# xh92117/Retinex-image-Enhancement

Hardware: AMD Instinct MI355X
Metric: images/sec at 512x512 bs=32 per GPU (UP-Retinex forward) (higher is better)
Workload: dtype f32; 1 GPU; configs[1]: bs=32/GPU 512x512 plain forward, fp32; global_batch=32, image_size=512, variant=plain, parallelism=batch-shard x1 (no data-path collective)

## Files before the change

### retinex-image-enhancement_amd/csrc/conv_ring.hip

```cpp
#include <algorithm>
#include <cstdlib>
#include <cstring>

#include "upr_common.h"

namespace upr {

typedef float f32x4_r __attribute__((ext_vector_type(4)));
typedef _Float16 f16x8_r __attribute__((ext_vector_type(8)));
typedef _Float16 f16x4_r __attribute__((ext_vector_type(4)));
typedef __attribute__((address_space(3))) void* lds_void_ptr_r;

__device__ __attribute__((aligned(256))) uint4 g_ring_zero[16];
__device__ __attribute__((aligned(256))) uint2 g_ring_sink[512 * 16];
__device__ __attribute__((aligned(256))) float g_ring_sink32[512 * 64];
__device__ __attribute__((aligned(256))) unsigned g_ring_ninf32[64] = {
#define NINF4 0xFF800000u, 0xFF800000u, 0xFF800000u, 0xFF800000u
    NINF4, NINF4, NINF4, NINF4, NINF4, NINF4, NINF4, NINF4, NINF4, NINF4, NINF4, NINF4, NINF4, NINF4, NINF4, NINF4
#undef NINF4
};
__device__ __attribute__((aligned(256))) unsigned g_ring_ninf[64] = {
#define NINF4 0xFC00FC00u, 0xFC00FC00u, 0xFC00FC00u, 0xFC00FC00u
    NINF4, NINF4, NINF4, NINF4, NINF4, NINF4, NINF4, NINF4, NINF4, NINF4, NINF4, NINF4, NINF4, NINF4, NINF4, NINF4
#undef NINF4
};

enum RingMode : int { kRingConv = 0, kRingHead = 1, kRingFam = 2, kRingS2 = 3 };
enum RingFlags : int {
  kRingRes = 1, kRingRelu = 2, kRingSc = 4, kRingOcc3 = 8, kRingWide = 16, kRingOut2 = 32, kRingOut32 = 64,
  kRingDil2 = 128, kRingResPre = 256, kRingPool = 512, kRingXPool = 1024, kRingR32 = 2048,
  kRingAblDma = 4096, kRingAblMma = 8192, kRingAblSt = 16384,
  kRingMma16 = 32768
};

template <int NPL, int RW_, int GROWS_, bool DEINT_ = false>
struct Ring {
  static constexpr int RW = RW_;
  static constexpr int GROWS = GROWS_;
  static constexpr int RR = 4 * GROWS;
  static constexpr int PLANE = RR * RW * 16;
  static constexpr int BYTES = NPL * PLANE;
  static constexpr int GPX = GROWS * RW;
  static constexpr int NI = (GPX + 63) / 64;
  static constexpr int PPW = NPL / 4;
  static constexpr int G = NI * PPW;
  static constexpr bool DEINT = DEINT_;
  static constexpr int HALF = (RW + 1) / 2;
  static_assert(NPL % 4 == 0, "planes are split over the 4 waves");
  static_assert((RR & (RR - 1)) == 0, "ring rows: power of two");
};

template <class R>
struct RingLanes {
  int dr[R::NI], col[R::NI], off[R::NI];
  __device__ __forceinline__ void init(int lane, int W, int cs) {
#pragma unroll
    for (int i = 0; i < R::NI; ++i) {
      const int q = i * 64 + lane;
      const int p = q % R::RW;
      dr[i] = q < R::GPX ? q / R::RW : -1;
      col[i] = R::DEINT ? (p < R::HALF ? 2 * p : 2 * (p - R::HALF) + 1) : p;
      off[i] = (dr[i] * W + col[i]) * cs;
    }
  }
  __device__ __forceinline__ void issue(const half_t* src, int cs, int b, int H, int W, int iy0, int ix0, bool live,
                                        const half_t* fill, unsigned char* ring, int grp, int wave) const {
    const half_t* base = src + ((long long)(b * H + iy0) * W + ix0) * cs;
#pragma unroll
    for (int i = 0; i < R::NI; ++i) {
      if (dr[i] >= 0) {
        const bool ok = live && (unsigned)(iy0 + dr[i]) < (unsigned)H && (unsigned)(ix0 + col[i]) < (unsigned)W;
        const half_t* p = ok ? base + off[i] : fill;
#pragma unroll
        for (int k = 0; k < R::PPW; ++k) {
          const int c = wave + 4 * k;
          __builtin_amdgcn_global_load_lds(p + c * 8, (lds_void_ptr_r)(ring + c * R::PLANE + grp * R::GPX * 16 + i * 1024),
                                           16, 0, 0);
        }
      }
    }
  }
};
// ... 640 lines not shown
        for (int nt = 0; nt < NT; ++nt)
#pragma unroll
          for (int i = 0; i < 4; ++i) {
            float v = pool[nt][i];
            v += __shfl_xor(v, 1);
            v += __shfl_xor(v, 2);
            v += __shfl_xor(v, 4);
            v += __shfl_xor(v, 8);
            if (fr == 0) pool_add(op.pool, (size_t)b * op.N + nt * 16 + fg * 4 + i, v);
            pool[nt][i] = 0.f;
          }
        flushed = true;
      }
    }
    advance(cc);
  }
  asm volatile("s_waitcnt vmcnt(0)" ::: "memory");
}

template <int CPP>
__device__ __forceinline__ int ring32_res_swz(int l) {
  if constexpr (CPP == 8) return (l >> 1) & 7;
  else return l & 15;
}

template <int MODE, int NB, int FL>
struct Ring32Cfg {
  static constexpr bool HEAD = MODE == kRingHead;
  static constexpr bool RES = FL & kRingRes, RELU = (FL & kRingRelu) != 0;
  static constexpr bool RESPRE = (FL & kRingResPre) != 0, POOL = (FL & kRingPool) != 0;
  static constexpr int DIL = (FL & kRingDil2) ? 2 : 1, HA = DIL;
  static constexpr bool XP = (FL & kRingXPool) != 0;
  static constexpr int C = 32, NT = NB / 16, NG = 2;
  using RA = Ring<8, 32 + 2 * HA, 4>;
  using RB = Ring<8, 34, 4>;
  static constexpr int NSL = XP ? 11 : 9;
  static constexpr bool WREG = NT == 2 || (NT == 4 && !RES);
  static constexpr bool M16 = (FL & kRingMma16) != 0;
  static_assert(!M16 || WREG, "split in registers: register-resident filters only");
  static constexpr bool TAPCH = M16 && NT == 4;
  static constexpr int WBYTES = TAPCH ? 9 * NT * 1024 : WREG ? 0 : 9 * NB * 32 * 4;
  static constexpr int EW = RES ? 32 * NB * 4 : HEAD ? 512 : 0;
  static constexpr int E = RES ? NB / 8 : HEAD ? 1 : 0;
  static constexpr int LDS = WBYTES + RA::BYTES + (XP ? RB::BYTES : 0) + 4 * EW;
  static constexpr int G = RA::G + (XP ? RB::G : 0);
  static constexpr int S = HEAD ? NG : NG * NT;
  static constexpr int W0 = G, W1 = E + G + S, WK = 2 * S + E + G, WF = WK + (POOL ? 4 * NT : 0);
  static_assert(WF <= 63, "vmcnt immediate");
  static_assert(!RESPRE || RES, "kRingResPre qualifies kRingRes");
  static_assert(!(HEAD && (POOL || DIL == 2)), "head: plain 3x3");
  static_assert(!XP || (WREG && DIL == 1 && !RES && !HEAD), "x / maxpool slices: the FAM h3 part");
};

template <int MODE, int NB, int FL>
__global__ __launch_bounds__(256) void conv_ring32_kernel(RingArgs a) {
  using K = Ring32Cfg<MODE, NB, FL>;
  using RA = typename K::RA;
  constexpr bool HEAD = K::HEAD, RES = K::RES;
  constexpr int NT = K::NT, NG = K::NG, HA = K::HA, DIL = K::DIL;
  using RB = typename K::RB;
  typedef float f32x4 __attribute__((ext_vector_type(4)));
  const ConvOp& op = a.op;
  extern __shared__ __attribute__((aligned(16))) unsigned char smem[];
  unsigned char* Wl = smem;
  unsigned char* ringA = smem + K::WBYTES;
  const int tid = threadIdx.x, lane = tid & 63;
  const int wave = __builtin_amdgcn_readfirstlane(tid >> 6);
  const int fr = lane & 15, fg = lane >> 4;
  unsigned char* ringB = ringA + RA::BYTES;
  unsigned char* epi = ringA + RA::BYTES + (K::XP ? RB::BYTES : 0) + wave * K::EW;
  const int H = op.Ho, W = op.Wo;
  const ConvSeg& sa = op.seg[0];
  const int per_xcd = gridDim.x >> 3;
  const int v0 = (blockIdx.x & 7) * per_xcd + (blockIdx.x >> 3);
  const int nu = v0 < a.nunits ? (a.nunits - 1 - v0) / (int)gridDim.x + 1 : 0;
  const int KT = nu * a.steps;

  constexpr bool M16 = K::M16;
  f32x4 wr[K::WREG && !M16 ? K::NSL : 1][NT][2];
  f16x8_t wh[M16 ? K::NSL : 1][NT], wl[M16 && !K::TAPCH ? K::NSL : 1][NT];
  int wsh[NT];
  if constexpr (M16) {
#pragma unroll
    for (int nt = 0; nt < NT; ++nt) {
      const float* row = (const float*)op.W + (size_t)(nt * 16 + fr) * op.Kpad + fg * 8;
      float mx = 0.f;
#pragma unroll
      for (int t = 0; t < K::NSL; ++t) {
        const f32x4 w0 = *(const f32x4*)(row + t * 32), w1 = *(const f32x4*)(row + t * 32 + 4);
#pragma unroll
        for (int i = 0; i < 4; ++i) mx = fmaxf(mx, fmaxf(__builtin_fabsf(w0[i]), __builtin_fabsf(w1[i])));
      }
      mx = fmaxf(mx, __shfl_xor(mx, 16));
      mx = fmaxf(mx, __shfl_xor(mx, 32));
      wsh[nt] = split_row_shift(mx);
      const float wsn = __builtin_ldexpf(1.f, wsh[nt]);
#pragma unroll
      for (int t = 0; t < K::NSL; ++t) {
        const f32x4 w0 = *(const f32x4*)(row + t * 32), w1 = *(const f32x4*)(row + t * 32 + 4);
        const float v[8] = {w0[0], w0[1], w0[2], w0[3], w1[0], w1[1], w1[2], w1[3]};
        if constexpr (K::TAPCH) {
          f16x8_t lo;
          split_w_f32x8(v, wsn, wh[t][nt], lo);
          if (wave == 0) *(f16x8_t*)(Wl + (t * NT + nt) * 1024 + lane * 16) = lo;
        } else {
          split_w_f32x8(v, wsn, wh[t][nt], wl[t][nt]);
        }
      }
    }
  } else if constexpr (K::WREG) {
#pragma unroll
// ... 11 lines not shown
  }
  const half_t* srcA = (const half_t*)((const float*)sa.src + sa.coff);
  const int csA = sa.cs * 2;
  const half_t* zero = (const half_t*)g_ring_zero;
  RingLanes<RA> la;
  la.init(lane, sa.Win, csA);
  const ConvSeg& sx = op.seg[K::XP ? 1 : 0];
  const half_t* srcB = (const half_t*)((const float*)sx.src + sx.coff);
  const int csB = sx.cs * 2;
  const half_t* ninf = (const half_t*)g_ring_ninf32;
  RingLanes<RB> lb;
  if constexpr (K::XP) lb.init(lane, sx.Win, csB);

  auto unit_of = [&](int j, int& b, int& y0, int& x0) {
    const int u = v0 + j * (int)gridDim.x;
    const int sx = u % a.nstrips, r = u / a.nstrips;
    b = r / a.nseg;
    y0 = (r % a.nseg) * a.rs;
    x0 = sx * 32;
  };
  const int S = a.steps - 1;
  struct Cursor {
    int j, s, b, y0, x0;
  };
  Cursor cc{0, -1, 0, 0, 0};
  if (nu > 0) unit_of(0, cc.b, cc.y0, cc.x0);
  Cursor dc = cc;
  auto advance = [&](Cursor& c) {
    if (++c.s == S) {
      c.s = -1;
      if (++c.j < nu) unit_of(c.j, c.b, c.y0, c.x0);
    }
  };
  auto issue = [&](int k) {
    const bool live = dc.j < nu;
    la.issue(srcA, csA, dc.b, sa.Hin, sa.Win, dc.y0 + 4 * dc.s + HA, dc.x0 - HA, live, zero, ringA, (k + 1) & 3, wave);
    if constexpr (K::XP)
      lb.issue(srcB, csB, dc.b, sx.Hin, sx.Win, dc.y0 + 4 * dc.s + 1, dc.x0 - 1, live, ninf, ringB, (k + 1) & 3, wave);
    advance(dc);
  };

  __syncthreads();
  issue(0);
  issue(1);

  float bv[NT][4];
#pragma unroll
  for (int nt = 0; nt < NT; ++nt)
#pragma unroll
    for (int i = 0; i < 4; ++i) bv[nt][i] = op.bias ? op.bias[nt * 16 + fg * 4 + i] : 0.f;
  int esh[M16 ? NT : 1];
  if constexpr (M16) {
#pragma unroll
    for (int nt = 0; nt < NT; ++nt) {
      esh[nt] = 0;
#pragma unroll
      for (int i = 0; i < 4; ++i) {
        const int sh = __shfl(wsh[nt], fg * 4 + i);
        esh[nt] |= (sh & 255) << (8 * i);
        bv[nt][i] = __builtin_ldexpf(bv[nt][i], sh);
      }
    }
  }
  float bad = 0.f;
  float hw2[NT][4];
  if constexpr (HEAD) {
#pragma unroll
    for (int nt = 0; nt < NT; ++nt)
#pragma unroll
      for (int i = 0; i < 4; ++i) hw2[nt][i] = op.head_w[nt * 16 + fg * 4 + i];
  }
  const int abase = 2 * fg * RA::PLANE + fr * 16;
  const int ocs = op.out_cs, rcs = RES ? (K::RESPRE ? op.res1_cs : op.res2_cs) : 0;
  const float* resp = RES ? (const float*)(K::RESPRE ? op.res1 : op.res2) : nullptr;
  const size_t HWs = (size_t)H * W;
  float pool[K::POOL ? NT : 1][4];
#pragma unroll
  for (int nt = 0; nt < (K::POOL ? NT : 1); ++nt)
#pragma unroll
    for (int i = 0; i < 4; ++i) pool[nt][i] = 0.f;
  bool flushed = false;

  for (int kk = 0; kk < KT; ++kk) {
    if (kk == 0) asm volatile("s_waitcnt vmcnt(%0)" ::"n"(K::W0) : "memory");
    else if (kk == 1) asm volatile("s_waitcnt vmcnt(%0)" ::"n"(K::W1) : "memory");
    else if (K::POOL && flushed) asm volatile("s_waitcnt vmcnt(%0)" ::"n"(K::WF) : "memory");
    else asm volatile("s_waitcnt vmcnt(%0)" ::"n"(K::WK) : "memory");
    __builtin_amdgcn_s_barrier();
    flushed = false;
    const int s = cc.s, b = cc.b, x0 = cc.x0;
    const int yend = min(H, cc.y0 + a.rs);
    const int y = cc.y0 + 4 * s + wave;
    const bool rowok = s >= 0 && y < yend;
    const size_t prow = (size_t)(b * H + (rowok ? y : 0)) * W + x0;
    bool ovalid[NG];
#pragma unroll
    for (int g = 0; g < NG; ++g) ovalid[g] = rowok && x0 + g * 16 + fr < W;
    if constexpr (RES) {
      constexpr int CPP = NB / 4;
#pragma unroll
      for (int i = 0; i < K::E; ++i) {
        const int q = i * 64 + lane, px = q / CPP;
        const bool ok = rowok && x0 + px < W;
        const void* p = ok ? (const void*)(resp + (prow + px) * rcs + ((q % CPP) ^ ring32_res_swz<CPP>(px)) * 4)
                           : (const void*)zero;
        __builtin_amdgcn_global_load_lds(p, (lds_void_ptr_r)(epi + i * 1024), 16, 0, 0);
      }
    }
    if constexpr (HEAD) {
      const int ppc = op.x_f16 ? 8 : 4, cpr = 32 / ppc;
      if (lane < 3 * cpr) {
        const int c = lane / cpr, k = lane % cpr;
        const bool ok = rowok && x0 + k * ppc < W;
        const size_t e = (size_t)b * 2 * HWs + prow + c * HWs + k * ppc;
        const void* p = !ok ? (const void*)zero
                            : op.x_f16 ? (const void*)((const half_t*)op.x_nchw + e) : (const void*)(op.x_nchw + e);
        __builtin_amdgcn_global_load_lds(p, (lds_void_ptr_r)epi, 16, 0, 0);
      }
    }
    issue(kk + 2);

    f32x4 acc[NT][NG];
#pragma unroll
    for (int nt = 0; nt < NT; ++nt)
#pragma unroll
      for (int g = 0; g < NG; ++g) acc[nt][g] = f32x4{bv[nt][0], bv[nt][1], bv[nt][2], bv[nt][3]};
    f32x4 acc2[M16 ? NT : 1][NG];
    if constexpr (M16) {
#pragma unroll
      for (int nt = 0; nt < NT; ++nt)
#pragma unroll
        for (int g = 0; g < NG; ++g) acc2[nt][g] = f32x4{0.f, 0.f, 0.f, 0.f};
    }
    auto mm16 = [&](int t, int g, const f32x4& x0, const f32x4& x1, const f16x8_t (&wlo)[NT]) {
      const float v[8] = {x0[0], x0[1], x0[2], x0[3], x1[0], x1[1], x1[2], x1[3]};
      f16x8_t xh, xl;
      split_f32x8(v, xh, xl);
#pragma unroll
      for (int nt = 0; nt < NT; ++nt) {
        acc[nt][g] = __builtin_amdgcn_mfma_f32_16x16x32_f16(wh[t][nt], xh, acc[nt][g], 0, 0, 0);
        acc[nt][g] = __builtin_amdgcn_mfma_f32_16x16x32_f16(wlo[nt], xh, acc[nt][g], 0, 0, 0);
        acc2[nt][g] = __builtin_amdgcn_mfma_f32_16x16x32_f16(wh[t][nt], xl, acc2[nt][g], 0, 0, 0);
      }
    };
#define RING_FENCE __builtin_amdgcn_sched_barrier(0)
#define RING_LDS_DONE                                                               \
  do {                                                                              \
    RING_FENCE;                                                                     \
    __builtin_amdgcn_s_waitcnt(0xC07F);  \
    RING_FENCE;                                                                     \
  } while (0)
    constexpr bool TAPCH = K::TAPCH;
    if constexpr (TAPCH) {
      if (s >= 0) {
        static_assert(NG == 2, "chunk index: tap * 2 + group");
        f32x4 tx[2][2];
        f16x8_t wlt[2][NT];
        auto ldt = [&](int c, f32x4 (&x)[2]) {
          const int r = (c >> 1) / 3, sc = (c >> 1) % 3, g = c & 1;
          const unsigned char* xr = ringA + abase + ((4 * kk + 4 + wave - HA + (r - 1) * DIL) & 15) * (RA::RW * 16) +
                                    (g * 16 + HA + (sc - 1) * DIL) * 16;
#pragma unroll
          for (int h = 0; h < 2; ++h) x[h] = *(const f32x4*)(xr + h * RA::PLANE);
          if (g == 0) {
#pragma unroll
            for (int nt = 0; nt < NT; ++nt)
              wlt[(c >> 1) & 1][nt] = *(const f16x8_t*)(Wl + ((c >> 1) * NT + nt) * 1024 + lane * 16);
          }
        };
        auto mmt = [&](int c, const f32x4 (&x)[2]) { mm16(c >> 1, c & 1, x[0], x[1], wlt[(c >> 1) & 1]); };
        ldt(0, tx[0]);
        ldt(1, tx[1]);
        RING_LDS_DONE;
        mmt(0, tx[0]);
#pragma unroll
        for (int c = 1; c < 18; ++c) {
          RING_FENCE;
          if (c + 1 < 18) ldt(c + 1, tx[(c + 1) & 1]);
          RING_FENCE;
          mmt(c, tx[c & 1]);
          RING_LDS_DONE;
        }
      }
    }
    if (s >= 0 && !TAPCH) {
      auto rowA = [&](int r) { return ((4 * kk + 4 + wave - HA + (r - 1) * DIL) & 15) * (RA::RW * 16); };
      constexpr int NW = K::WREG ? 1 : 3;
      f32x4 bx[2][3][NG][2], bw[2][NW][NT][2];
      auto ld = [&](int r, f32x4 (&x)[3][NG][2], f32x4 (&w)[NW][NT][2]) {
        const unsigned char* xr = ringA + abase + rowA(r);
#pragma unroll
        for (int sc = 0; sc < 3; ++sc)
#pragma unroll
          for (int g = 0; g < NG; ++g)
#pragma unroll
            for (int h = 0; h < 2; ++h)
              x[sc][g][h] = *(const f32x4*)(xr + h * RA::PLANE + (g * 16 + HA + (sc - 1) * DIL) * 16);
        if constexpr (!K::WREG) {
#pragma unroll
          for (int sc = 0; sc < 3; ++sc)
#pragma unroll
            for (int nt = 0; nt < NT; ++nt)
#pragma unroll
              for (int h = 0; h < 2; ++h)
                w[sc][nt][h] = *(const f32x4*)(Wl + ((size_t)((r * 3 + sc) * NB + nt * 16 + fr) * 32 + fg * 8 + h * 4) * 4);
        }
      };
      auto mm = [&](int r, const f32x4 (&x)[3][NG][2], const f32x4 (&w)[NW][NT][2]) {
        if constexpr (M16) {
#pragma unroll
          for (int sc = 0; sc < 3; ++sc)
#pragma unroll
            for (int g = 0; g < NG; ++g) mm16(r * 3 + sc, g, x[sc][g][0], x[sc][g][1], wl[r * 3 + sc]);
          return;
        }
#pragma unroll
        for (int sc = 0; sc < 3; ++sc)
#pragma unroll
          for (int j = 0; j < 8; ++j)
#pragma unroll
            for (int g = 0; g < NG; ++g)
#pragma unroll
              for (int nt = 0; nt < NT; ++nt) {
                const float wv = K::WREG ? wr[r * 3 + sc][nt][j >> 2][j & 3] : w[K::WREG ? 0 : sc][nt][j >> 2][j & 3];
                acc[nt][g] = __builtin_amdgcn_mfma_f32_16x16x4f32(wv, x[sc][g][j >> 2][j & 3], acc[nt][g], 0, 0, 0);
              }
      };
      ld(0, bx[0], bw[0]);
      ld(1, bx[1], bw[1]);
      RING_LDS_DONE;
      mm(0, bx[0], bw[0]);
      RING_FENCE;
      ld(2, bx[0], bw[0]);
      RING_FENCE;
      mm(1, bx[1], bw[1]);
      RING_LDS_DONE;
      if constexpr (K::XP) {
        const int bbase = 2 * fg * RB::PLANE + fr * 16;
        auto rowB = [&](int dy) { return ((4 * kk + 4 + wave - 1 + dy) & 15) * (RB::RW * 16); };
        f32x4 xr3[3][NG][2];
#pragma unroll
        for (int sc = 0; sc < 3; ++sc)
#pragma unroll
          for (int g = 0; g < NG; ++g)
#pragma unroll
            for (int h = 0; h < 2; ++h)
              xr3[sc][g][h] = *(const f32x4*)(ringB + bbase + rowB(-1) + h * RB::PLANE + (g * 16 + sc) * 16);
        RING_FENCE;
        mm(2, bx[0], bw[0]);
        RING_LDS_DONE;
        f32x4 ctr[NG][2], mx[NG][2];
#pragma unroll
        for (int g = 0; g < NG; ++g)
#pragma unroll
          for (int h = 0; h < 2; ++h)
            mx[g][h] = __builtin_elementwise_max(__builtin_elementwise_max(xr3[0][g][h], xr3[1][g][h]), xr3[2][g][h]);
#pragma unroll
        for (int dr = 1; dr < 3; ++dr) {
#pragma unroll
          for (int sc = 0; sc < 3; ++sc)
#pragma unroll
            for (int g = 0; g < NG; ++g)
#pragma unroll
              for (int h = 0; h < 2; ++h)
                xr3[sc][g][h] = *(const f32x4*)(ringB + bbase + rowB(dr - 1) + h * RB::PLANE + (g * 16 + sc) * 16);
          RING_LDS_DONE;
#pragma unroll
          for (int g = 0; g < NG; ++g)
#pragma unroll
            for (int h = 0; h < 2; ++h) {
              mx[g][h] = __builtin_elementwise_max(
                  mx[g][h], __builtin_elementwise_max(__builtin_elementwise_max(xr3[0][g][h], xr3[1][g][h]), xr3[2][g][h]));
              if (dr == 1) ctr[g][h] = xr3[1][g][h];
            }
        }
        if constexpr (M16) {
#pragma unroll
          for (int g = 0; g < NG; ++g) {
            mm16(9, g, ctr[g][0], ctr[g][1], wl[K::XP ? 9 : 0]);
            mm16(10, g, mx[g][0], mx[g][1], wl[K::XP ? 10 : 0]);
          }
        } else {
#pragma unroll
        for (int j = 0; j < 8; ++j)
#pragma unroll
          for (int g = 0; g < NG; ++g)
#pragma unroll
            for (int nt = 0; nt < NT; ++nt) {
              acc[nt][g] = __builtin_amdgcn_mfma_f32_16x16x4f32(wr[9][nt][j >> 2][j & 3], ctr[g][j >> 2][j & 3],
                                                                acc[nt][g], 0, 0, 0);
              acc[nt][g] = __builtin_amdgcn_mfma_f32_16x16x4f32(wr[10][nt][j >> 2][j & 3], mx[g][j >> 2][j & 3],
                                                                acc[nt][g], 0, 0, 0);
            }
        }
      } else {
        mm(2, bx[0], bw[0]);
      }
    }
#undef RING_LDS_DONE
#undef RING_FENCE

    asm volatile("s_waitcnt vmcnt(%0)" ::"n"(K::G) : "memory");
    if constexpr (M16) {
#pragma unroll
      for (int nt = 0; nt < NT; ++nt)
#pragma unroll
        for (int g = 0; g < NG; ++g)
#pragma unroll
          for (int i = 0; i < 4; ++i) {
            const float v = __builtin_fmaf(acc2[nt][g][i], kSplitLoInv, acc[nt][g][i]);
            bad = __builtin_fmaf(ovalid[g] ? v : 0.f, 0.f, bad);
            acc[nt][g][i] = __builtin_ldexpf(v, -(int)(signed char)(esh[nt] >> (8 * i)));
          }
    }
    if constexpr (HEAD) {
#pragma unroll
      for (int g = 0; g < NG; ++g) {
        float part = 0.f;
#pragma unroll
        for (int nt = 0; nt < NT; ++nt)
#pragma unroll
          for (int i = 0; i < 4; ++i) part += fmaxf(acc[nt][g][i], 0.f) * hw2[nt][i];
        part += __shfl_xor(part, 16);
        part += __shfl_xor(part, 32);
        const int xp = g * 16 + fr;
        float x0f, x1f, x2f;
        if (op.x_f16) {
          const half_t* xl = (const half_t*)epi;
          x0f = (float)xl[xp];
          x1f = (float)xl[32 + xp];
          x2f = (float)xl[64 + xp];
        } else {
          const float* xl = (const float*)epi;
// ... 19 lines not shown
          if constexpr (K::RELU) {
#pragma unroll
            for (int i = 0; i < 4; ++i) v[i] = fmaxf(v[i], 0.f);
          }
          if constexpr (RES && !K::RESPRE)
            v += *(const f32x4*)(epi + (g * 16 + fr) * NB * 4 + (((nt * 4 + fg) ^ ring32_res_swz<NB / 4>(fr)) * 16));
          if constexpr (K::POOL) {
#pragma unroll
            for (int i = 0; i < 4; ++i)
              if (ovalid[g]) pool[nt][i] += v[i];
          }
          *(f32x4*)(dg + nt * 16) = v;
        }
      }
    }
    if constexpr (K::POOL) {
      if (s == a.steps - 2) {
#pragma unroll
        for (int nt = 0; nt < NT; ++nt)
#pragma unroll
          for (int i = 0; i < 4; ++i) {
            float v = pool[nt][i];
            v += __shfl_xor(v, 1);
            v += __shfl_xor(v, 2);
            v += __shfl_xor(v, 4);
            v += __shfl_xor(v, 8);
            if (fr == 0) pool_add(op.pool, (size_t)cc.b * op.N + nt * 16 + fg * 4 + i, v);
            pool[nt][i] = 0.f;
          }
        flushed = true;
      }
    }
    advance(cc);
  }
  asm volatile("s_waitcnt vmcnt(0)" ::: "memory");
  if constexpr (M16) {
    if (bad != bad && op.ovf) *op.ovf = 1u;
  }
}

static int ring_cus() {
  static int cus = 0;
  if (!cus) {
    int dev = 0;
    if (hipGetDevice(&dev) != hipSuccess ||
        hipDeviceGetAttribute(&cus, hipDeviceAttributeMultiprocessorCount, dev) != hipSuccess || cus <= 0)
      cus = 256;
  }
  return cus;
}

static void ring_bands(RingArgs& a, const ConvOp& op, int grid) {
  const int per_band = op.B * a.nstrips;
  long best = -1;
  for (int nb = 1; nb <= 16; ++nb) {
    int rs = (cdiv(op.Ho, nb) + 3) / 4 * 4;
    if (rs < 8) rs = 8;
    const int nseg = cdiv(op.Ho, rs);
    const long cost = (long)cdiv(per_band * nseg, grid) * (rs / 4 + 1);
    if (best < 0 || cost < best) {
      best = cost;
      a.rs = rs;
      a.nseg = nseg;
    }
  }
  a.nunits = per_band * a.nseg;
// ... 115 lines not shown
  if (op.res2 && op.res2_cs % 4) return kErrUnsupported;
  const bool res = op.res2 != nullptr;
  if (s.stride == 2) {
    if (op.nseg != 1 || res || s.C != 32 || op.N != 64) return kErrUnsupported;
    if (s.Hin != 2 * op.Ho || s.Win != 2 * op.Wo) return kErrUnsupported;
    return ring_relu<kRingS2, 32, 64, 0>(op, st);
  }
  if (s.stride != 1 || s.Hin != op.Ho || s.Win != op.Wo) return kErrUnsupported;
  if (op.nseg == 2) {
    const ConvSeg& q = op.seg[1];
    if (s.C != 64 || op.N != 64 || res) return kErrUnsupported;
    if (q.kh != 1 || q.kw != 1 || q.stride != 2 || q.pad != 0 || q.pre != kPreNone || q.C != 32 || q.kbase != 576)
      return kErrUnsupported;
    if (q.Hin != 2 * op.Ho || q.Win != 2 * op.Wo || q.cs % 8 || q.coff % 8 || (uintptr_t)q.src % 16 || op.Kpad != 608)
      return kErrUnsupported;
    if (op.out2) return ring_relu<kRingConv, 64, 64, kRingSc | kRingOut2>(op, st);
    return ring_relu<kRingConv, 64, 64, kRingSc>(op, st);
  }
  if (op.nseg != 1) return kErrUnsupported;
  if (s.C == 32 && op.N == 32) {
    if (res) return ring_relu<kRingConv, 32, 32, kRingRes>(op, st);
    if (op.Wo >= 48) return ring_relu<kRingConv, 32, 32, kRingWide>(op, st);
    return ring_relu<kRingConv, 32, 32, kRingOcc3>(op, st);
  }
  if (s.C == 32 && op.N == 64) return res ? ring_relu<kRingConv, 32, 64, kRingRes>(op, st) : ring_relu<kRingConv, 32, 64, 0>(op, st);
  if (s.C == 64 && op.N == 64) return res ? ring_relu<kRingConv, 64, 64, kRingRes>(op, st) : ring_relu<kRingConv, 64, 64, 0>(op, st);
  return kErrUnsupported;
}

template <int MODE, int NB, int FL>
static int ring32_form(const ConvOp& op, hipStream_t st) {
  if constexpr (Ring32Cfg<MODE, NB, FL>::WREG) {
    if (op.mma16) {
      const int rc = launch_ring32_cfg<MODE, NB, FL | kRingMma16>(op, st);
      if (rc == kOk) conv_set_last_form(2);
      return rc;
    }
  }
  if (op.mma16 == 2) return kErrUnsupported;
  return launch_ring32_cfg<MODE, NB, FL>(op, st);
}

template <int MODE, int NB, int FL>
static int ring32_relu(const ConvOp& op, hipStream_t st) {
  return op.relu ? ring32_form<MODE, NB, FL | kRingRelu>(op, st) : ring32_form<MODE, NB, FL>(op, st);
}

int launch_conv_ring32(const ConvOp& op, hipStream_t st) {
  if (op.Ho < 4 || op.Wo < 16) return kErrUnsupported;
  const ConvSeg& s = op.seg[0];
  if (op.nseg == 3) {
    const ConvSeg& x1 = op.seg[1];
    const ConvSeg& x2 = op.seg[2];
    if (op.Kpad != 352 || op.N != 32 || op.store != kStoreNHWC || op.relu || op.pool || op.res1 || op.res2 ||
        op.img_bias || op.scale || op.out_cs % 4 || op.out_coff % 4)
      return kErrUnsupported;
    if (!ring_seg_ok(s) || s.C != 32 || s.stride != 1 || s.Hin != op.Ho || s.Win != op.Wo || s.cs % 4 || s.coff % 4)
      return kErrUnsupported;
    for (const ConvSeg* q : {&x1, &x2})
      if (q->kh != 1 || q->kw != 1 || q->stride != 1 || q->pad != 0 || q->C != 32 || q->Hin != op.Ho ||
          q->Win != op.Wo || q->src != x1.src || q->cs != x1.cs || q->coff != x1.coff)
        return kErrUnsupported;
    if (x1.pre != kPreNone || x2.pre != kPreMaxPool3 || x1.kbase != 288 || x2.kbase != 320 || x1.cs % 4 ||
        x1.coff % 4 || (uintptr_t)x1.src % 16)
      return kErrUnsupported;
    return ring32_form<kRingConv, 32, kRingXPool>(op, st);
  }
// ... 32 lines not shown
```

### retinex-image-enhancement_amd/csrc/model.hip

```cpp
#include <algorithm>
#include <atomic>
#include <cmath>
#include <cstdio>
#include <cstdlib>
#include <cstring>
#include <map>
#include <memory>
#include <mutex>
#include <string>
#include <vector>

#include "upr_common.h"
#include "../../include/upr.h"

namespace upr {

int launch_prep(const void* x, void* x2p, void* x3p, int B, int H, int W, int dtype, hipStream_t st);
int launch_preact_f16(const void* x, const float* sc, const float* sh, void* o, size_t npix, int C, hipStream_t st);
int launch_conv3(const void* x, const float* w, const float* bias, void* out0, void* out1, int B, int h, int wd,
                 int dtype, hipStream_t st, void* out2 = nullptr, const float* ps = nullptr,
                 const float* ph = nullptr);
int launch_fam_ca(const float* pool, const float* w1, const float* b1, const float* w2, const float* b2, float* ca,
                  int B, int HW, hipStream_t st);
int launch_fam_mix(const void* y, const float* ca, const float* P, float* mm, float* p, int B, int HW, int dtype,
// ... 316 lines not shown
  int dtype = 0;
  int use_preact = 0, use_aspp = 0, flags = 0;
  void* dev_blob = nullptr;
  size_t blob_bytes = 0;
  std::vector<upr::GemmLayer> layers;
  std::vector<upr::Op> ops;
  bool prof = false;
  std::vector<std::vector<hipEvent_t>> ev_pending;
  std::vector<hipEvent_t> ev_free;
  std::vector<double> st_ms, st_flops, st_bytes;
  std::vector<int> st_calls;
  std::vector<double> cur_flops, cur_bytes;
  int side_begin = -1, side_end = -1;
  struct Side {
    hipStream_t s = nullptr;
    hipEvent_t fork = nullptr, join = nullptr;
    unsigned long long last_use = 0;
    ~Side() {
      if (s) (void)hipStreamSynchronize(s);
      if (join) (void)hipEventDestroy(join);
      if (fork) (void)hipEventDestroy(fork);
      if (s) (void)hipStreamDestroy(s);
    }
  };
  static constexpr size_t kMaxSides = 16;
  std::map<std::pair<int, hipStream_t>, std::shared_ptr<Side>> sides;
  unsigned long long side_clock = 0;
  std::mutex sides_mu;
  std::atomic<long long> forks{0};
  std::atomic<int> split_state{0};
  unsigned* ovf_dev = nullptr;
  volatile unsigned* ovf_host = nullptr;
  int split_regs = 0;
  int split_w64 = 0;
  std::vector<int> op_forms;
  std::mutex forms_mu;
};

namespace upr {

struct BufGeom {
  int C;
  int shift;
  int is_f32;
  int pyramid;
};

static BufGeom buf_geom(int id, int use_aspp) {
  switch (id) {
    case B_X2P: return {3, 2, 0, 1};
    case B_X3P: return {3, 4, 0, 2};
    case B_X1: case B_S1IN: return {32, 0, 0, 0};
    case B_S2IN: return {32, 2, 0, 1};
    case B_S3IN: return {32, 4, 0, 2};
    case B_E1T: case B_X2: return {64, 1, 0, 0};
    case B_E2T: case B_X3: return {128, 2, 0, 0};
    case B_E3T: case B_X4: case B_B0T: case B_B0: case B_AP: case B_B1T: case B_X5: return {256, 3, 0, 0};
    case B_ASPP: return {use_aspp ? 1024 : 0, 3, 0, 0};
    case B_U3: case B_V3: case B_D3: return {128, 2, 0, 0};
    case B_U2: case B_V2: case B_D2: return {64, 1, 0, 0};
    case B_U1: case B_V1: case B_D1: return {32, 0, 0, 0};
    case B_H1: return {64, 0, 0, 0};
    case B_Y1: return {32, 0, 0, 0};
    case B_H2: return {64, 2, 0, 1};
    case B_Y2: return {32, 2, 0, 1};
    case B_H3: return {64, 4, 0, 2};
// ... 639 lines not shown
        c.scale = nullptr;
        c.bias = L.bias != SIZE_MAX ? fptr(L.bias) : nullptr;
        c.img_bias = o.img_bias ? ib : nullptr;
        c.res1 = o.res1 >= 0 ? buf(o.res1) : nullptr; c.res1_cs = o.res1_cs;
        c.relu = o.relu;
        c.res2 = o.res2 >= 0 ? buf(o.res2) : nullptr; c.res2_cs = o.res2_cs;
        c.store = o.store;
        if (o.store == kStoreHeadIllu) {
          c.head_w = fptr(o.head_w); c.head_b = o.head_b;
          c.x_nchw = (const float*)x; c.x_f16 = dt == kF16;
          c.illu = illu32; c.illu_f16 = 0;
          c.out = nullptr;
        } else {
          c.out = buf(o.out); c.out_cs = o.out_cs; c.out_coff = o.out_coff;
        }
        c.pool = o.pool_slot >= 0 ? pool + (size_t)o.pool_slot * B * 256 * kPoolEntryFloats : nullptr;
        if (o.out2 >= 0) {
          c.out2 = buf(o.out2); c.out2_cs = L.N;
          c.pre2_scale = fptr(o.ps); c.pre2_shift = fptr(o.ph);
        }
        if (split_now && o.split_layer >= 0) {
          rc = launch_conv_wide(split_op(o, ho, wo), st);
          forms[oi] = 1;
        } else {
          rc = kErrUnsupported;
          if (regs_now && dt == kF32 && o.w64_w != SIZE_MAX) {
            ConvOp cw = c;
            cw.W = blob + o.w64_w; cw.scale = fptr(o.w64_scale);
            cw.mma16 = 3; cw.ovf = m->ovf_dev;
            rc = launch_conv_wsplit(cw, st);
            if (rc == kOk) forms[oi] = 3;
          }
          if (rc == kErrUnsupported) {
            if (regs_now && dt == kF32) { c.mma16 = 1; c.ovf = m->ovf_dev; }
            rc = launch_conv(c, dt, st);
            forms[oi] = conv_last_form();
          }
        }
        if (m->prof) {
          const double Mpx = (double)B * ho * wo;
          double K = 0, bytes = (double)L.N * L.Kpad * elt;
          for (int i = 0; i < c.nseg; ++i) {
            K += (double)c.seg[i].kh * c.seg[i].kw * c.seg[i].C;
            bytes += (double)B * c.seg[i].Hin * c.seg[i].Win * c.seg[i].C * elt;
          }
          const double nout = o.store == kStoreHeadIllu ? 1.0 : (double)L.N;
          bytes += Mpx * nout * (o.store == kStoreHeadIllu ? 4.0 : elt);
          if (c.res1) bytes += Mpx * L.N * elt;
          if (c.res2) bytes += Mpx * L.N * elt;
          if (c.out2) bytes += Mpx * L.N * elt;
          m->cur_flops[oi] = 2.0 * Mpx * L.N * K;
          m->cur_bytes[oi] = bytes;
        }
        break;
      }
      case OP_PREACT: {
        int h, w;
        lvl_dims(o.level, h, w);
        const int C = buf_geom(o.out, m->use_aspp).C;
        rc = launch_preact_f16(buf(o.in), fptr(o.w), fptr(o.b), buf(o.out), (size_t)B * h * w, C, st);
        if (m->prof) m->cur_bytes[oi] = 2.0 * B * h * w * C * elt;
        break;
      }
      case OP_SPLIT: {
        if (!split_now) break;
        int h, w;
        lvl_dims(o.level, h, w);
// ... 133 lines not shown
  typedef _Float16 h8 __attribute__((ext_vector_type(8)));
  const size_t i = (size_t)blockIdx.x * blockDim.x + threadIdx.x;
  if (i >= n8) return;
  const size_t pix = i / C8;
  const int c = (int)(i - pix * C8) * 8;
  const half_t* sp = x + pix * (size_t)(16 * C8) + c;
  const h8 h = *(const h8*)sp, l = *(const h8*)(sp + 8 * C8);
  f4 a, b;
#pragma unroll
  for (int e = 0; e < 4; ++e) {
    a[e] = (float)h[e] + (float)l[e] * kSplitLoInv;
    b[e] = (float)h[e + 4] + (float)l[e + 4] * kSplitLoInv;
  }
  *(f4*)(y + i * 8) = a;
  *(f4*)(y + i * 8 + 4) = b;
}
int launch_split_f32(const float* x, void* y, size_t npix, int C, unsigned* ovf, hipStream_t st) {
  if (C <= 0 || C % 8 || ((uintptr_t)x | (uintptr_t)y) % 16) return kErrArg;
  const size_t n8 = npix * (size_t)(C / 8);
  if (n8 == 0) return kOk;
  if ((n8 + 255) / 256 > 0x7fffffffull) return kErrShape;
  hipLaunchKernelGGL(split_f32_kernel, dim3((unsigned)((n8 + 255) / 256)), dim3(256), 0, st, x, (half_t*)y, n8, C / 8, ovf);
  return (int)hipGetLastError();
}
int launch_unsplit_f32(const void* x, float* y, size_t npix, int C, hipStream_t st) {
  if (C <= 0 || C % 8 || ((uintptr_t)x | (uintptr_t)y) % 16) return kErrArg;
  const size_t n8 = npix * (size_t)(C / 8);
  if (n8 == 0) return kOk;
  if ((n8 + 255) / 256 > 0x7fffffffull) return kErrShape;
  hipLaunchKernelGGL(unsplit_f32_kernel, dim3((unsigned)((n8 + 255) / 256)), dim3(256), 0, st, (const half_t*)x, y, n8, C / 8);
  return (int)hipGetLastError();
}

}

using namespace upr;

extern "C" {

int upr_model_create(const UprTensorDesc* params, int n_params, int use_preact, int use_aspp, int dtype, int flags,
                     UprModel** out) {
  if (!out || (n_params > 0 && !params) || (dtype != UPR_F32 && dtype != UPR_F16)) return UPR_ERR_ARG;
  *out = nullptr;
  constexpr int kKnownFlags = UPR_MODEL_IENET_ONLY | UPR_MODEL_HEAD_ONLY;
  if ((flags & ~kKnownFlags) || (flags & kKnownFlags) == kKnownFlags) return UPR_ERR_ARG;
  ParamSet P;
  for (int i = 0; i < n_params; ++i) {
    const UprTensorDesc& d = params[i];
    if (!d.name || d.ndim < 0 || d.ndim > 4) return UPR_ERR_ARG;
    HostTensor t;
    int64_t n = 1;
    for (int k = 0; k < d.ndim; ++k) { t.shape.push_back(d.shape[k]); n *= d.shape[k]; }
    if (n > 0 && !d.data) return UPR_ERR_ARG;
    t.v.assign(d.data, d.data + n);
    P.t[d.name] = std::move(t);
  }
  std::unique_ptr<UprModel> m(new UprModel());
  m->dtype = dtype; m->use_preact = use_preact ? 1 : 0; m->use_aspp = use_aspp ? 1 : 0; m->flags = flags;
  const char* se = getenv("UPR_FP32_SPLIT");
  const bool split_env = !(se && *se && atoi(se) == 0);
  if (split_env && dtype == UPR_F32 && !m->use_preact && !m->use_aspp) m->split_state.store(1);
  const char* sr = getenv("UPR_FP32_SPLIT_REGS");
  m->split_regs = !(sr && *sr && atoi(sr) == 0);
  const char* sw = getenv("UPR_FP32_SPLIT_W64");
  m->split_w64 = !(sw && *sw && atoi(sw) == 0);
  int rc = build_model(m.get(), P);
  if (rc == kOk && m->split_state.load() == 1) {
    hipError_t e = hipMalloc((void**)&m->ovf_dev, 256);
    if (e == hipSuccess) e = hipMemset(m->ovf_dev, 0, 256);
    if (e == hipSuccess) e = hipHostMalloc((void**)&m->ovf_host, sizeof(unsigned), hipHostMallocDefault);
    if (e == hipSuccess) *m->ovf_host = 0u;
    else rc = (int)e;
  }
  if (rc != kOk) {
    if (m->dev_blob) (void)hipFree(m->dev_blob);
    if (m->ovf_dev) (void)hipFree(m->ovf_dev);
    if (m->ovf_host) (void)hipHostFree((void*)m->ovf_host);
    return rc;
  }
  *out = m.release();
  return UPR_OK;
}

size_t upr_model_workspace(const UprModel* model, int B, int H, int W) {
  if (!model || B <= 0 || H <= 0 || W <= 0) return 0;
  return ws_layout(model, B, H, W, nullptr);
}

int upr_model_forward(UprModel* model, const void* x, int B, int H, int W, void* enh, void* refl, void* illu,
                      void* workspace, size_t workspace_bytes, void* stream) {
  const bool head_only = (model && (model->flags & UPR_MODEL_HEAD_ONLY));
  if (!model || !x || (!illu && !head_only) || B <= 0) return UPR_ERR_ARG;
  if (!(model->flags & UPR_MODEL_IENET_ONLY) && (!enh || !refl)) return UPR_ERR_ARG;
  if (H % 8 || W % 8 || H < 16 || W < 16) return UPR_ERR_SHAPE;
  if ((long long)B * H * W > (1LL << 31) / 32) return UPR_ERR_SHAPE;
  const size_t need = ws_layout(model, B, H, W, nullptr);
// ... 119 lines not shown
  }
  c.nseg = 1;
  ConvSeg& s = c.seg[0];
  s.src = x; s.C = Cin; s.cs = Cin; s.coff = 0; s.Hin = H; s.Win = W;
  s.kh = kh; s.kw = kw; s.stride = stride; s.pad = pad; s.dil = dil; s.pre = kPreNone; s.kbase = 0;
  c.B = B; c.Ho = Ho; c.Wo = Wo; c.N = Cout; c.Kpad = kh * kw * Cin;
  c.W = w; c.bias = bias; c.relu = relu;
  if (relu) { c.res1 = residual; c.res1_cs = Cout; }
  else { c.res2 = residual; c.res2_cs = Cout; }
  c.out = y; c.out_cs = Cout; c.out_coff = 0; c.store = kStoreNHWC;
  return launch_conv(c, dtype, (hipStream_t)stream);
}

int upr_conv2d_nhwc_regs(const void* x, int B, int H, int W, int Cin, const void* w, const float* bias, int Cout,
                         int kh, int kw, int stride, int pad, int dil, const void* residual, int relu, void* y,
                         unsigned* overflow, void* stream) {
  if (!x || !w || !y || B <= 0 || H <= 0 || W <= 0 || Cin % 32 || Cout % 32 || Cin <= 0 || Cout <= 0) return UPR_ERR_ARG;
  if (kh <= 0 || kw <= 0 || stride <= 0 || dil <= 0 || pad < 0) return UPR_ERR_ARG;
  const int Ho = (H + 2 * pad - dil * (kh - 1) - 1) / stride + 1;
  const int Wo = (W + 2 * pad - dil * (kw - 1) - 1) / stride + 1;
  if (Ho <= 0 || Wo <= 0) return UPR_ERR_SHAPE;
  ConvOp c;
  memset(&c, 0, sizeof(c));
  c.nseg = 1;
  ConvSeg& s = c.seg[0];
  s.src = x; s.C = Cin; s.cs = Cin; s.coff = 0; s.Hin = H; s.Win = W;
  s.kh = kh; s.kw = kw; s.stride = stride; s.pad = pad; s.dil = dil; s.pre = kPreNone; s.kbase = 0;
  c.B = B; c.Ho = Ho; c.Wo = Wo; c.N = Cout; c.Kpad = kh * kw * Cin;
  c.W = w; c.bias = bias; c.relu = relu;
  if (relu && residual) return UPR_ERR_UNSUPPORTED;
  c.res2 = residual; c.res2_cs = Cout;
  c.out = y; c.out_cs = Cout; c.out_coff = 0; c.store = kStoreNHWC;
  c.mma16 = 1; c.ovf = overflow;
  return launch_conv_regs(c, (hipStream_t)stream);
}

size_t upr_pack_split_f32(const float* w, int Cout, int Cin, int kh, int kw, void* out, size_t out_bytes) {
  if (!w || Cout <= 0 || Cin <= 0 || Cin % 64 || kh <= 0 || kw <= 0) return 0;
  std::vector<SegWeights> segs(1);
  segs[0].spec = seg(0, Cin, Cin, 0, kh, 1, 0, 1);
  segs[0].spec.kw = kw;
  segs[0].w.assign(w, w + (size_t)Cout * Cin * kh * kw);
  SplitPack sp;
  if (!pack_split(Cout, segs, sp)) return 0;
  const size_t wbytes = align_up(sp.W.size() * 2, 256), need = wbytes + sp.scale.size() * 4;
  if (out && out_bytes >= need) {
    memset(out, 0, need);
    memcpy(out, sp.W.data(), sp.W.size() * 2);
    memcpy((uint8_t*)out + wbytes, sp.scale.data(), sp.scale.size() * 4);
  }
  return need;
}

static size_t split_w_bytes(int Cout, int K, size_t* scale_off) {
  const size_t wbytes = align_up((size_t)Cout * K * 4, 256);
  if (scale_off) *scale_off = wbytes;
  return wbytes + (size_t)Cout * 4;
}

size_t upr_pack_split_w_f32(const float* w, int Cout, int Cin, int kh, int kw, const float* w2, int C2, void* out,
                            size_t out_bytes) {
  if (!w || Cout <= 0 || Cout % 64 || Cin <= 0 || Cin % 32 || kh <= 0 || kw <= 0) return 0;
  if ((w2 != nullptr) != (C2 > 0) || C2 < 0 || C2 % 32) return 0;
  const int K1 = kh * kw * Cin, K = K1 + C2;
  std::vector<float> rows((size_t)Cout * K);
  for (int n = 0; n < Cout; ++n) {
// ... 62 lines not shown
```

### retinex-image-enhancement_amd/csrc/upr_common.h

```cpp
#pragma once
#include <hip/hip_runtime.h>
#include <stdint.h>
#include <stddef.h>

#define UPR_CHECK_HIP(expr)                                  \
  do {                                                       \
    hipError_t _e = (expr);                                  \
    if (_e != hipSuccess) return (int)_e;                    \
  } while (0)

namespace upr {

typedef _Float16 half_t;

enum : int {
  kOk = 0,
  kErrArg = -1,
  kErrShape = -2,
  kErrMissingParam = -3,
  kErrWorkspace = -4,
  kErrUnsupported = -5,
};

enum DType : int { kF32 = 0, kF16 = 1 };
// ... 26 lines not shown
  ConvSeg seg[4];
  int B, Ho, Wo, N;
  int Kpad;
  const void* W;
  const float* scale;
  const float* bias;
  const float* img_bias;
  const void* res1; int res1_cs;
  int relu;
  const void* res2; int res2_cs;
  void* out; int out_cs, out_coff;
  int store;
  float* pool;
  const float* head_w;
  float head_b;
  const float* x_nchw;
  int x_f16;
  float* illu;
  int illu_f16;
  void* out2; int out2_cs;
  const float* pre2_scale;
  const float* pre2_shift;
  float* out32; int out32_cs, out32_coff;
  const float* res32; int res32_cs;
  void* out32_h16; int out32_h16_cs;
  const void* mask16; int mask16_cs; int skip32;
  int out_s2;
  int krot;
  void* split_out; int split_cs, split_lo;
  float* out_f32; int out_f32_cs;
  int split_res;
  int mma16;
  unsigned* ovf;
};

constexpr float kSplitLoScale = 2048.f;
constexpr float kSplitLoInv = 1.f / 2048.f;

#ifdef __HIPCC__
typedef _Float16 f16x8_t __attribute__((ext_vector_type(8)));
__device__ __forceinline__ void split_f32x8(const float (&v)[8], f16x8_t& hi, f16x8_t& lo) {
#pragma unroll
  for (int i = 0; i < 8; ++i) {
    const half_t h = (half_t)v[i];
    hi[i] = h;
    lo[i] = (half_t)__builtin_fmaf((float)h, -kSplitLoScale, v[i] * kSplitLoScale);
  }
}
__device__ __forceinline__ void split_w_f32x8(const float (&v)[8], float s, f16x8_t& hi, f16x8_t& lo) {
#pragma unroll
  for (int i = 0; i < 8; ++i) {
    const float w = v[i] * s;
    const half_t h = (half_t)w;
    hi[i] = h;
    lo[i] = (half_t)(w - (float)h);
  }
}
#endif
__host__ __device__ inline int split_row_shift(float mx) {
  int sh = 0;
  if (mx > 0.f && mx < __builtin_inff()) {
    int e;
    (void)__builtin_frexpf(mx, &e);
    sh = 15 - e;
    sh = sh < -100 ? -100 : sh > 100 ? 100 : sh;
  }
// ... 47 lines not shown
```

Before: 2208 images/s.

## Split ring activations to fp16 hi/lo in LDS once, with a deeper ring

In the split-fp16 ring convolution, each staged fp32 activation group is now converted to hi/lo fp16 pairs once, in place in LDS. Previously every tap's MFMA call redid that split in registers. For the 32-channel plain conv form, the ring gets a fifth group with a load lead of three, so conversion of the next group can be interleaved with the current tap MFMAs. The other forms convert the whole group up front behind an extra barrier. The trade is more LDS use and occupancy pressure, extra waits and barriers, plus more complex ring indexing with a non-power-of-two ring.

```diff
diff --git a/retinex-image-enhancement_amd/csrc/conv_ring.hip b/retinex-image-enhancement_amd/csrc/conv_ring.hip
--- a/retinex-image-enhancement_amd/csrc/conv_ring.hip
+++ b/retinex-image-enhancement_amd/csrc/conv_ring.hip
@@ -1,6 +1,7 @@
 #include <algorithm>
 #include <cstdlib>
 #include <cstring>
+#include <type_traits>
 
 #include "upr_common.h"
 
@@ -30,14 +31,16 @@
   kRingRes = 1, kRingRelu = 2, kRingSc = 4, kRingOcc3 = 8, kRingWide = 16, kRingOut2 = 32, kRingOut32 = 64,
   kRingDil2 = 128, kRingResPre = 256, kRingPool = 512, kRingXPool = 1024, kRingR32 = 2048,
   kRingAblDma = 4096, kRingAblMma = 8192, kRingAblSt = 16384,
-  kRingMma16 = 32768
+  kRingMma16 = 32768,
+  kRingLds = 65536, kRingLdsTop = 131072
 };
 
-template <int NPL, int RW_, int GROWS_, bool DEINT_ = false>
+template <int NPL, int RW_, int GROWS_, bool DEINT_ = false, int NGRP_ = 4>
 struct Ring {
   static constexpr int RW = RW_;
   static constexpr int GROWS = GROWS_;
-  static constexpr int RR = 4 * GROWS;
+  static constexpr int NGRP = NGRP_;
+  static constexpr int RR = NGRP * GROWS;
   static constexpr int PLANE = RR * RW * 16;
   static constexpr int BYTES = NPL * PLANE;
   static constexpr int GPX = GROWS * RW;
@@ -47,7 +50,7 @@
   static constexpr bool DEINT = DEINT_;
   static constexpr int HALF = (RW + 1) / 2;
   static_assert(NPL % 4 == 0, "planes are split over the 4 waves");
-  static_assert((RR & (RR - 1)) == 0, "ring rows: power of two");
+  static_assert(NGRP != 4 || (RR & (RR - 1)) == 0, "ring rows: power of two");
 };
 
 template <class R>
@@ -754,8 +757,13 @@
   static constexpr int DIL = (FL & kRingDil2) ? 2 : 1, HA = DIL;
   static constexpr bool XP = (FL & kRingXPool) != 0;
   static constexpr int C = 32, NT = NB / 16, NG = 2;
-  using RA = Ring<8, 32 + 2 * HA, 4>;
+  static constexpr bool LS = (FL & kRingLds) != 0, LSA = LS && !(FL & kRingLdsTop);
+  static_assert(!LS || (FL & kRingMma16), "split in LDS: a form of the split-fp16 programs");
+  static_assert(LS || !(FL & kRingLdsTop), "kRingLdsTop qualifies kRingLds");
+  static constexpr int NGRP = LSA ? 5 : 4, LEAD = LSA ? 3 : 2;
+  using RA = Ring<8, 32 + 2 * HA, 4, false, NGRP>;
   using RB = Ring<8, 34, 4>;
+  static constexpr int NCV = (4 * RA::GPX + 255) / 256;
   static constexpr int NSL = XP ? 11 : 9;
   static constexpr bool WREG = NT == 2 || (NT == 4 && !RES);
   static constexpr bool M16 = (FL & kRingMma16) != 0;
@@ -769,6 +777,7 @@
   static constexpr int S = HEAD ? NG : NG * NT;
   static constexpr int W0 = G, W1 = E + G + S, WK = 2 * S + E + G, WF = WK + (POOL ? 4 * NT : 0);
   static_assert(WF <= 63, "vmcnt immediate");
+  static_assert(!LS || LDS <= 160 * 1024, "the deeper ring fits one block per CU");
   static_assert(!RESPRE || RES, "kRingResPre qualifies kRingRes");
   static_assert(!(HEAD && (POOL || DIL == 2)), "head: plain 3x3");
   static_assert(!XP || (WREG && DIL == 1 && !RES && !HEAD), "x / maxpool slices: the FAM h3 part");
@@ -799,6 +808,8 @@
   const int KT = nu * a.steps;
 
   constexpr bool M16 = K::M16;
+  using RingCvt = std::integral_constant<bool, K::LS>;
+  static_assert(K::NCV <= 3, "one conversion item per tap row");
   f32x4 wr[K::WREG && !M16 ? K::NSL : 1][NT][2];
   f16x8_t wh[M16 ? K::NSL : 1][NT], wl[M16 && !K::TAPCH ? K::NSL : 1][NT];
   int wsh[NT];
@@ -876,17 +887,35 @@
       if (++c.j < nu) unit_of(c.j, c.b, c.y0, c.x0);
     }
   };
-  auto issue = [&](int k) {
+  Cursor dcx = cc;
+  auto issue = [&](int ga, int gx) {
     const bool live = dc.j < nu;
-    la.issue(srcA, csA, dc.b, sa.Hin, sa.Win, dc.y0 + 4 * dc.s + HA, dc.x0 - HA, live, zero, ringA, (k + 1) & 3, wave);
-    if constexpr (K::XP)
-      lb.issue(srcB, csB, dc.b, sx.Hin, sx.Win, dc.y0 + 4 * dc.s + 1, dc.x0 - 1, live, ninf, ringB, (k + 1) & 3, wave);
+    la.issue(srcA, csA, dc.b, sa.Hin, sa.Win, dc.y0 + 4 * dc.s + HA, dc.x0 - HA, live, zero, ringA, ga, wave);
+    if constexpr (K::XP && K::LEAD == 2)
+      lb.issue(srcB, csB, dc.b, sx.Hin, sx.Win, dc.y0 + 4 * dc.s + 1, dc.x0 - 1, live, ninf, ringB, gx, wave);
     advance(dc);
   };
+  auto issue_x = [&](int gx) {
+    if constexpr (K::XP && K::LEAD == 3) {
+      lb.issue(srcB, csB, dcx.b, sx.Hin, sx.Win, dcx.y0 + 4 * dcx.s + 1, dcx.x0 - 1, dcx.j < nu, ninf, ringB, gx, wave);
+      advance(dcx);
+    }
+  };
+  int cvoff[K::LS ? K::NCV : 1];
+  if constexpr (K::LS) {
+#pragma unroll
+    for (int j = 0; j < K::NCV; ++j) {
+      const int q = j * 256 + tid;
+      cvoff[j] = q < 4 * RA::GPX ? 2 * (q / RA::GPX) * RA::PLANE + (q % RA::GPX) * 16 : -1;
+    }
+  }
 
   __syncthreads();
-  issue(0);
-  issue(1);
+  issue(1, 1);
+  issue_x(1);
+  issue(2, 2);
+  issue_x(2);
+  if constexpr (K::LEAD == 3) issue(3, 0);
 
   float bv[NT][4];
 #pragma unroll
@@ -923,14 +952,25 @@
   for (int nt = 0; nt < (K::POOL ? NT : 1); ++nt)
 #pragma unroll
     for (int i = 0; i < 4; ++i) pool[nt][i] = 0.f;
-  bool flushed = false;
+  bool flushed = false, flushed2 = false;
+  int gb = 0;
 
   for (int kk = 0; kk < KT; ++kk) {
+    auto grp_at = [&](int d) {
+      if constexpr (K::NGRP == 4) return (kk + d) & 3;
+      else return gb + d >= K::NGRP ? gb + d - K::NGRP : gb + d;
+    };
+    auto ring_row = [&](int c) {
+      if constexpr (K::NGRP == 4) return (4 * kk + c) & 15;
+      else return 4 * gb + c >= RA::RR ? 4 * gb + c - RA::RR : 4 * gb + c;
+    };
+    if constexpr (K::LS) __builtin_amdgcn_s_waitcnt(0xC07F);
     if (kk == 0) asm volatile("s_waitcnt vmcnt(%0)" ::"n"(K::W0) : "memory");
     else if (kk == 1) asm volatile("s_waitcnt vmcnt(%0)" ::"n"(K::W1) : "memory");
-    else if (K::POOL && flushed) asm volatile("s_waitcnt vmcnt(%0)" ::"n"(K::WF) : "memory");
+    else if (K::POOL && (flushed || (K::LEAD == 3 && flushed2))) asm volatile("s_waitcnt vmcnt(%0)" ::"n"(K::WF) : "memory");
     else asm volatile("s_waitcnt vmcnt(%0)" ::"n"(K::WK) : "memory");
     __builtin_amdgcn_s_barrier();
+    flushed2 = flushed;
     flushed = false;
     const int s = cc.s, b = cc.b, x0 = cc.x0;
     const int yend = min(H, cc.y0 + a.rs);
@@ -962,7 +1002,49 @@
         __builtin_amdgcn_global_load_lds(p, (lds_void_ptr_r)epi, 16, 0, 0);
       }
     }
-    issue(kk + 2);
+    issue(grp_at(K::LEAD + 1), (kk + 3) & 3);
+    issue_x((kk + 3) & 3);
+
+    f32x4 ct[K::LS ? K::NCV : 1][2];
+    auto cv_on = [&](int j) { return (j + 1) * 256 <= 4 * RA::GPX || cvoff[K::LS ? j : 0] >= 0; };
+    auto cv_read = [&](int grp) {
+      if constexpr (K::LS) {
+#pragma unroll
+        for (int j = 0; j < K::NCV; ++j)
+          if (cv_on(j)) {
+            const unsigned char* p = ringA + grp * (RA::GPX * 16) + cvoff[j];
+            ct[j][0] = *(const f32x4*)p;
+            ct[j][1] = *(const f32x4*)(p + RA::PLANE);
+          }
+      }
+    };
+    auto cv_write = [&](int grp, int j) {
+      if constexpr (K::LS) {
+        if (cv_on(j)) {
+          unsigned char* p = ringA + grp * (RA::GPX * 16) + cvoff[j];
+          const float v[8] = {ct[j][0][0], ct[j][0][1], ct[j][0][2], ct[j][0][3],
+                              ct[j][1][0], ct[j][1][1], ct[j][1][2], ct[j][1][3]};
+          f16x8_t hi, lo;
+          split_f32x8(v, hi, lo);
+          *(f16x8_t*)p = hi;
+          *(f16x8_t*)(p + RA::PLANE) = lo;
+        }
+      }
+    };
+    auto cv_group = [&](int grp) {
+      cv_read(grp);
+#pragma unroll
+      for (int j = 0; j < K::NCV; ++j) cv_write(grp, j);
+    };
+    const int cvg = grp_at(K::LSA ? 2 : 1);
+    if constexpr (K::LSA) {
+      if (kk == 0) cv_group(1);
+      cv_read(cvg);
+    } else if constexpr (K::LS) {
+      cv_group(cvg);
+      __builtin_amdgcn_s_waitcnt(0xC07F);
+      __builtin_amdgcn_s_barrier();
+    }
 
     f32x4 acc[NT][NG];
 #pragma unroll
@@ -976,10 +1058,15 @@
 #pragma unroll
         for (int g = 0; g < NG; ++g) acc2[nt][g] = f32x4{0.f, 0.f, 0.f, 0.f};
     }
-    auto mm16 = [&](int t, int g, const f32x4& x0, const f32x4& x1, const f16x8_t (&wlo)[NT]) {
-      const float v[8] = {x0[0], x0[1], x0[2], x0[3], x1[0], x1[1], x1[2], x1[3]};
+    auto mm16 = [&](auto cvt, int t, int g, const f32x4& x0, const f32x4& x1, const f16x8_t (&wlo)[NT]) {
       f16x8_t xh, xl;
-      split_f32x8(v, xh, xl);
+      if constexpr (decltype(cvt)::value) {
+        xh = __builtin_bit_cast(f16x8_t, x0);
+        xl = __builtin_bit_cast(f16x8_t, x1);
+      } else {
+        const float v[8] = {x0[0], x0[1], x0[2], x0[3], x1[0], x1[1], x1[2], x1[3]};
+        split_f32x8(v, xh, xl);
+      }
 #pragma unroll
       for (int nt = 0; nt < NT; ++nt) {
         acc[nt][g] = __builtin_amdgcn_mfma_f32_16x16x32_f16(wh[t][nt], xh, acc[nt][g], 0, 0, 0);
@@ -1002,7 +1089,7 @@
         f16x8_t wlt[2][NT];
         auto ldt = [&](int c, f32x4 (&x)[2]) {
           const int r = (c >> 1) / 3, sc = (c >> 1) % 3, g = c & 1;
-          const unsigned char* xr = ringA + abase + ((4 * kk + 4 + wave - HA + (r - 1) * DIL) & 15) * (RA::RW * 16) +
+          const unsigned char* xr = ringA + abase + ring_row(4 + wave - HA + (r - 1) * DIL) * (RA::RW * 16) +
                                     (g * 16 + HA + (sc - 1) * DIL) * 16;
 #pragma unroll
           for (int h = 0; h < 2; ++h) x[h] = *(const f32x4*)(xr + h * RA::PLANE);
@@ -1012,7 +1099,7 @@
               wlt[(c >> 1) & 1][nt] = *(const f16x8_t*)(Wl + ((c >> 1) * NT + nt) * 1024 + lane * 16);
           }
         };
-        auto mmt = [&](int c, const f32x4 (&x)[2]) { mm16(c >> 1, c & 1, x[0], x[1], wlt[(c >> 1) & 1]); };
+        auto mmt = [&](int c, const f32x4 (&x)[2]) { mm16(RingCvt{}, c >> 1, c & 1, x[0], x[1], wlt[(c >> 1) & 1]); };
         ldt(0, tx[0]);
         ldt(1, tx[1]);
         RING_LDS_DONE;
@@ -1023,12 +1110,13 @@
           if (c + 1 < 18) ldt(c + 1, tx[(c + 1) & 1]);
           RING_FENCE;
           mmt(c, tx[c & 1]);
+          if (K::LSA && c <= K::NCV) cv_write(cvg, c - 1);
           RING_LDS_DONE;
         }
       }
     }
     if (s >= 0 && !TAPCH) {
-      auto rowA = [&](int r) { return ((4 * kk + 4 + wave - HA + (r - 1) * DIL) & 15) * (RA::RW * 16); };
+      auto rowA = [&](int r) { return ring_row(4 + wave - HA + (r - 1) * DIL) * (RA::RW * 16); };
       constexpr int NW = K::WREG ? 1 : 3;
       f32x4 bx[2][3][NG][2], bw[2][NW][NT][2];
       auto ld = [&](int r, f32x4 (&x)[3][NG][2], f32x4 (&w)[NW][NT][2]) {
@@ -1055,7 +1143,8 @@
 #pragma unroll
           for (int sc = 0; sc < 3; ++sc)
 #pragma unroll
-            for (int g = 0; g < NG; ++g) mm16(r * 3 + sc, g, x[sc][g][0], x[sc][g][1], wl[r * 3 + sc]);
+            for (int g = 0; g < NG; ++g) mm16(RingCvt{}, r * 3 + sc, g, x[sc][g][0], x[sc][g][1], wl[r * 3 + sc]);
+          if (K::LSA && r < K::NCV) cv_write(cvg, r);
           return;
         }
 #pragma unroll
@@ -1121,8 +1210,8 @@
         if constexpr (M16) {
 #pragma unroll
           for (int g = 0; g < NG; ++g) {
-            mm16(9, g, ctr[g][0], ctr[g][1], wl[K::XP ? 9 : 0]);
-            mm16(10, g, mx[g][0], mx[g][1], wl[K::XP ? 10 : 0]);
+            mm16(std::false_type{}, 9, g, ctr[g][0], ctr[g][1], wl[K::XP ? 9 : 0]);
+            mm16(std::false_type{}, 10, g, mx[g][0], mx[g][1], wl[K::XP ? 10 : 0]);
           }
         } else {
 #pragma unroll
@@ -1143,6 +1232,12 @@
     }
 #undef RING_LDS_DONE
 #undef RING_FENCE
+    if constexpr (K::LSA) {
+      if (s < 0) {
+#pragma unroll
+        for (int j = 0; j < K::NCV; ++j) cv_write(cvg, j);
+      }
+    }
 
     asm volatile("s_waitcnt vmcnt(%0)" ::"n"(K::G) : "memory");
     if constexpr (M16) {
@@ -1228,6 +1323,7 @@
       }
     }
     advance(cc);
+    if constexpr (K::NGRP != 4) gb = gb + 1 == K::NGRP ? 0 : gb + 1;
   }
   asm volatile("s_waitcnt vmcnt(0)" ::: "memory");
   if constexpr (M16) {
@@ -1409,7 +1505,11 @@
 static int ring32_form(const ConvOp& op, hipStream_t st) {
   if constexpr (Ring32Cfg<MODE, NB, FL>::WREG) {
     if (op.mma16) {
-      const int rc = launch_ring32_cfg<MODE, NB, FL | kRingMma16>(op, st);
+      constexpr bool AHEAD = MODE == kRingConv && NB == 32 && !(FL & (kRingDil2 | kRingXPool));
+      const int form = op.ring_split ? op.ring_split : AHEAD ? 3 : 2;
+      const int rc = form == 1   ? launch_ring32_cfg<MODE, NB, FL | kRingMma16>(op, st)
+                     : form == 2 ? launch_ring32_cfg<MODE, NB, FL | kRingMma16 | kRingLds | kRingLdsTop>(op, st)
+                                 : launch_ring32_cfg<MODE, NB, FL | kRingMma16 | kRingLds>(op, st);
       if (rc == kOk) conv_set_last_form(2);
       return rc;
     }
diff --git a/retinex-image-enhancement_amd/csrc/model.hip b/retinex-image-enhancement_amd/csrc/model.hip
--- a/retinex-image-enhancement_amd/csrc/model.hip
+++ b/retinex-image-enhancement_amd/csrc/model.hip
@@ -372,6 +372,7 @@
   unsigned* ovf_dev = nullptr;
   volatile unsigned* ovf_host = nullptr;
   int split_regs = 0;
+  int ring_split = 0;
   int split_w64 = 0;
   std::vector<int> op_forms;
   std::mutex forms_mu;
@@ -1077,7 +1078,7 @@
             if (rc == kOk) forms[oi] = 3;
           }
           if (rc == kErrUnsupported) {
-            if (regs_now && dt == kF32) { c.mma16 = 1; c.ovf = m->ovf_dev; }
+            if (regs_now && dt == kF32) { c.mma16 = 1; c.ovf = m->ovf_dev; c.ring_split = m->ring_split; }
             rc = launch_conv(c, dt, st);
             forms[oi] = conv_last_form();
           }
@@ -1277,6 +1278,13 @@
   return (int)hipGetLastError();
 }
 
+static int ring_split_env() {
+  const char* e = getenv("UPR_RING_SPLIT_LDS");
+  if (!e || !*e) return 0;
+  const int v = atoi(e);
+  return v == 0 ? 1 : v == 2 || v == 3 ? v : 0;
+}
+
 }
 
 using namespace upr;
@@ -1307,6 +1315,7 @@
   if (split_env && dtype == UPR_F32 && !m->use_preact && !m->use_aspp) m->split_state.store(1);
   const char* sr = getenv("UPR_FP32_SPLIT_REGS");
   m->split_regs = !(sr && *sr && atoi(sr) == 0);
+  m->ring_split = ring_split_env();
   const char* sw = getenv("UPR_FP32_SPLIT_W64");
   m->split_w64 = !(sw && *sw && atoi(sw) == 0);
   int rc = build_model(m.get(), P);
@@ -1492,6 +1501,7 @@
   c.res2 = residual; c.res2_cs = Cout;
   c.out = y; c.out_cs = Cout; c.out_coff = 0; c.store = kStoreNHWC;
   c.mma16 = 1; c.ovf = overflow;
+  c.ring_split = ring_split_env();
   return launch_conv_regs(c, (hipStream_t)stream);
 }
 
diff --git a/retinex-image-enhancement_amd/csrc/upr_common.h b/retinex-image-enhancement_amd/csrc/upr_common.h
--- a/retinex-image-enhancement_amd/csrc/upr_common.h
+++ b/retinex-image-enhancement_amd/csrc/upr_common.h
@@ -82,6 +82,7 @@
   int split_res;
   int mma16;
   unsigned* ovf;
+  int ring_split;
 };
 
 constexpr float kSplitLoScale = 2048.f;
```

After: 2310 images/s, median of 6. 4.6% higher.
